# XuyangBai/PointDSC

Hardware: NVIDIA H100
Metric: correspondence-sets/sec (PointDSC.forward, N=1000, B=256) (higher is better)
Workload: dtype fp16 hi/lo split (3 products) with f32 accumulate

## Files before the change

pointdsc_b200/csrc/nsm.cu:

```cuda
#include <cuda_fp16.h>

#include "common.cuh"
#include "kernels.h"
#include "sets.cuh"
#include "warp_select.cuh"

namespace pdsc {

__global__ void gather_rows_kernel(const float* __restrict__ normed, const int32_t* __restrict__ seeds,
                                   float* __restrict__ out, const SetDesc* __restrict__ sets) {
  const int b = blockIdx.y, s = blockIdx.x, lane = threadIdx.x;
  const SetDesc d = sets[b];
  if (s >= d.S) return;
  int idx = seeds[(size_t)d.seed0 + s];
  idx = min(max(idx, 0), d.N - 1);
  const float4 v = *reinterpret_cast<const float4*>(normed + ((size_t)d.row0 + idx) * kC + lane * 4);
  *reinterpret_cast<float4*>(out + ((size_t)d.seed0 + s) * kC + lane * 4) = v;
}
void launch_gather_rows(const float* normed, const int32_t* seeds, float* out, int B, int N, int S, cudaStream_t st,
                        const SetDesc* sets) {
  if (S <= 0) return;
  gather_rows_kernel<<<dim3(S, B), 32, 0, st>>>(normed, seeds, out, sets);
}


__global__ void __launch_bounds__(256) knn_select_kernel(const float* __restrict__ dist, int32_t* __restrict__ knn_idx,
                                                         const SetDesc* __restrict__ sets, int nsets, int rows, int warps_per_cta,
                                                         int NPmax, int Pmax) {
  extern __shared__ __align__(16) unsigned char knn_smem[];
  const int lane = threadIdx.x & 31, warp = threadIdx.x >> 5;
  const int row = blockIdx.x * warps_per_cta + warp;
  if (row >= rows) return;
  const SetDesc sd = sets[find_set(nsets, row, [&](int b) { return sets[b].seed0; })];
  const int s = row - sd.seed0, N = sd.N, k = sd.k;
  int P = 2;
  while (P < k + 1) P <<= 1;
  const float* d = dist + sd.dist0 + (size_t)s * N;
  int32_t* out = knn_idx + sd.knn0 + (size_t)s * k;
  const int NP = (N + 31) & ~31;
  const size_t per_warp = (size_t)NPmax * 4 + 1024 + (size_t)Pmax * 8;
  unsigned char* base = knn_smem + (size_t)warp * per_warp;
  unsigned long long* sel = reinterpret_cast<unsigned long long*>(base);
  uint32_t* hist = reinterpret_cast<uint32_t*>(base + (size_t)Pmax * 8);
  uint32_t* keys = hist + 256;
  if ((N & 3) == 0 && (reinterpret_cast<uintptr_t>(d) & 15) == 0) {
    const uint32_t kbase = (uint32_t)__cvta_generic_to_shared(keys);
    for (int j4 = lane; j4 < (N >> 2); j4 += 32)
      asm volatile("cp.async.cg.shared.global [%0], [%1], 16;" ::"r"(kbase + (uint32_t)j4 * 16u), "l"(d + 4 * j4) : "memory");
    asm volatile("cp.async.wait_all;" ::: "memory");
  } else {
    for (int j0 = lane; j0 < N; j0 += 256) {
      float t[8];
#pragma unroll
      for (int q = 0; q < 8; ++q) t[q] = (j0 + 32 * q < N) ? d[j0 + 32 * q] : 0.f;
#pragma unroll
      for (int q = 0; q < 8; ++q)
        if (j0 + 32 * q < N) keys[j0 + 32 * q] = __float_as_uint(t[q]);
    }
  }
  __syncwarp();
  for (int j = lane; j < NP; j += 32) keys[j] = j < N ? dist_key32(__uint_as_float(keys[j])) : 0xFFFFFFFFu;
  __syncwarp();
  warp_select_sorted(keys, hist, sel, N, NP, k + 1, P, lane);
  for (int r = 1 + lane; r <= k; r += 32) {
    const unsigned long long v = sel[r];
    out[r - 1] = (v == ~0ull || (uint32_t)(v >> 32) == 0xFFFFFFFFu) ? 0 : (int32_t)(v & 0xFFFFFFFFull);
  }
}

void launch_knn_select(const float* dist, int32_t* knn_idx, int B, int N, int S, int k, cudaStream_t st,
                       const SetDesc* sets, int total_seeds) {
  if (S <= 0) return;
  const int rows = total_seeds;
  int P = 2;
  while (P < k + 1) P <<= 1;
  const int NP = (N + 31) & ~31;
  const size_t per_warp = (size_t)NP * 4 + 1024 + (size_t)P * 8;
  int warps = (int)((200 * 1024) / per_warp);
  warps = warps > 8 ? 8 : (warps < 1 ? 1 : warps);
  const int smem = (int)(per_warp * warps);
  ensure_dynamic_smem(reinterpret_cast<const void*>(knn_select_kernel), smem);
  knn_select_kernel<<<(rows + warps - 1) / warps, warps * 32, smem, st>>>(dist, knn_idx, sets, B, rows, warps, NP, P);
}

__device__ __forceinline__ void cp_async_16(uint32_t dst_smem, const void* src) {
  asm volatile("cp.async.cg.shared.global [%0], [%1], 16;" ::"r"(dst_smem), "l"(src) : "memory");
}
__device__ __forceinline__ void cp_async_wait_all() { asm volatile("cp.async.wait_all;" ::: "memory"); }

template <int WPS>
__device__ __forceinline__ void seed_group_sync() {
  if (WPS == 1) __syncwarp();
  else __syncthreads();
}

template <int WPS, int RI, int CW>
__device__ __forceinline__ uint32_t power_iteration_regs(const float* M, int ms, int k, float* v, float* red, float* it_out,
                                                         int iters, int tg) {
  constexpr int RG = 8 * WPS;
  const int lane = tg & 31, warp = tg >> 5;
  const int rg = tg >> 2, cq = tg & 3;
  const int CQ = (k + 3) >> 2;
  const int c_lo = cq * CQ, c_hi = min(k, c_lo + CQ);
  float m[RI][CW], vq[CW], vrow[RI];
#pragma unroll
  for (int i = 0; i < RI; ++i) {
    const int row = rg + RG * i;
#pragma unroll
    for (int c = 0; c < CW; ++c) m[i][c] = (row < k && c_lo + c < c_hi) ? M[row * ms + c_lo + c] : 0.f;
    vrow[i] = 1.0f;
  }
#pragma unroll
  for (int c = 0; c < CW; ++c) vq[c] = (c_lo + c < c_hi) ? 1.0f : 0.f;
  uint32_t mask = 0u;
  for (int t = 0; t < iters; ++t) {
    float u[RI], ss = 0.f;
#pragma unroll
    for (int i = 0; i < RI; ++i) {
      float p = 0.f;
#pragma unroll
      for (int c = 0; c < CW; ++c) p = fmaf(m[i][c], vq[c], p);
      p += __shfl_xor_sync(0xffffffffu, p, 1);
      p += __shfl_xor_sync(0xffffffffu, p, 2);
      u[i] = p;
      ss += (rg + RG * i < k) ? p * p : 0.f;
    }
    ss += __shfl_xor_sync(0xffffffffu, ss, 4);
    ss += __shfl_xor_sync(0xffffffffu, ss, 8);
    ss += __shfl_xor_sync(0xffffffffu, ss, 16);
    if (WPS > 1) {
      if (lane == 0) red[warp] = ss;
      __syncthreads();
      ss = ((red[0] + red[1]) + red[2]) + red[3];
    }
    const float nrm = sqrtf(ss) + 1e-6f;
    bool ok = true;
#pragma unroll
    for (int i = 0; i < RI; ++i) {
      const int row = rg + RG * i;
      const float vn = u[i] / nrm;
      ok = ok && (row >= k || fabsf(vn - vrow[i]) <= 1e-8f + 1e-5f * fabsf(vrow[i]));
      vrow[i] = vn;
      if (row < k && cq == 0) {
        v[row] = vn;
        it_out[(size_t)t * k + row] = vn;
      }
    }
    bool all_ok = __all_sync(0xffffffffu, ok);
    if (WPS > 1) {
      if (lane == 0) red[4 + warp] = all_ok ? 1.f : 0.f;
      __syncthreads();
      all_ok = (red[4] + red[5] + red[6] + red[7]) == 4.f;
    } else {
      __syncwarp();
    }
    if (all_ok) mask |= (1u << t);
#pragma unroll
    for (int c = 0; c < CW; ++c) vq[c] = (c_lo + c < c_hi) ? v[c_lo + c] : 0.f;
    if (WPS == 1) __syncwarp();
  }
  return mask;
}

template <int WPS>
__global__ void __launch_bounds__(WPS == 1 ? 256 : 128) nsm_power_kernel(
    const float* __restrict__ normed, const float* __restrict__ src, const float* __restrict__ tgt,
    const int32_t* __restrict__ knn_idx, float* __restrict__ iterates, uint32_t* __restrict__ conv_mask,
    float* __restrict__ compat_out, const SetDesc* sets, int k_lo, int k_hi, int iters, float sigma2, float sigmad2,
    int mask_stride, int groups_per_cta, int per_group_floats) {
  const float rc_sigma2 = 1.0f / sigma2, rc_sigmad2 = 1.0f / sigmad2;
  extern __shared__ __align__(16) float sm[];
  constexpr int TS = 32 * WPS;
  const int lane = threadIdx.x & 31, warp = threadIdx.x >> 5;
  const int group = (WPS == 1) ? warp : 0;
  const int tg = (WPS == 1) ? lane : (int)threadIdx.x;
  const int b = blockIdx.y;
  const SetDesc d = sets[b];
  const int N = d.N, S = d.S, k = d.k;
  if (k < k_lo || k > k_hi) return;
  const int s = blockIdx.x * groups_per_cta + group;
  if (s >= S) return;
  const int ms = k | 1;
  const int kp = (k + 3) & ~3;
  float* F = sm + (size_t)group * per_group_floats;
  float* M = F + (size_t)kp * 32;
  float* pa = M + (size_t)k * ms;
  float* pb = pa + k * 3;
  float* v = pb + k * 3;
  int* idx = reinterpret_cast<int*>(v + k);
  float* red = reinterpret_cast<float*>(idx + k);
  const size_t nb0 = (size_t)d.knn0 + (size_t)s * k;

  for (int a = tg; a < k; a += TS) {
    int j = knn_idx[nb0 + a];
    j = min(max(j, 0), N - 1);
    idx[a] = j;
    const float* ps = src + ((size_t)d.row0 + j) * 3;
    const float* pt = tgt + ((size_t)d.row0 + j) * 3;
    pa[a * 3 + 0] = ps[0]; pa[a * 3 + 1] = ps[1]; pa[a * 3 + 2] = ps[2];
    pb[a * 3 + 0] = pt[0]; pb[a * 3 + 1] = pt[1]; pb[a * 3 + 2] = pt[2];
    v[a] = 1.0f;
    M[a * ms + a] = 0.0f;
  }
  seed_group_sync<WPS>();

  const int nb = kp >> 2;
  const int nblk = nb * (nb + 1) / 2;
  constexpr int kMaxRounds = 2;
  const uint32_t f_base = (uint32_t)__cvta_generic_to_shared(F);
  for (int r0 = 0; r0 * TS < nblk; r0 += kMaxRounds) {
    int bA[kMaxRounds], bB[kMaxRounds];
    float acc[kMaxRounds][4][4];
#pragma unroll
    for (int r = 0; r < kMaxRounds; ++r) {
      const int t = tg + TS * (r0 + r);
      int A = 0, rem = t < nblk ? t : 0;
      while (rem >= nb - A) { rem -= nb - A; ++A; }
      bA[r] = A; bB[r] = A + rem;
#pragma unroll
      for (int i = 0; i < 4; ++i)
#pragma unroll
        for (int j = 0; j < 4; ++j) acc[r][i][j] = 0.f;
    }
#pragma unroll 1
    for (int quarter = 0; quarter < 4; ++quarter) {
      const int q = tg & 7;
      for (int a = tg >> 3; a < kp; a += TS / 8) {
        const uint32_t dst = f_base + (uint32_t)((a * 32 + ((q ^ ((a >> 2) & 7)) << 2)) * 4);
        if (a < k) cp_async_16(dst, normed + ((size_t)d.row0 + idx[a]) * kC + quarter * 32 + q * 4);
        else *reinterpret_cast<float4*>(F + a * 32 + ((q ^ ((a >> 2) & 7)) << 2)) = make_float4(0.f, 0.f, 0.f, 0.f);
      }
      cp_async_wait_all();
      seed_group_sync<WPS>();
#pragma unroll
      for (int r = 0; r < kMaxRounds; ++r) {
        if (tg + TS * (r0 + r) < nblk) {
          const float* xa = F + (size_t)(4 * bA[r]) * 32;
          const float* yb = F + (size_t)(4 * bB[r]) * 32;
          const int sx = bA[r] & 7, sy = bB[r] & 7;
#pragma unroll 2
          for (int cc = 0; cc < 8; ++cc) {
            float4 x[4], y[4];
#pragma unroll
            for (int i = 0; i < 4; ++i) {
              x[i] = *reinterpret_cast<const float4*>(xa + i * 32 + ((cc ^ sx) << 2));
              y[i] = *reinterpret_cast<const float4*>(yb + i * 32 + ((cc ^ sy) << 2));
            }
#pragma unroll
            for (int i = 0; i < 4; ++i)
#pragma unroll
              for (int j = 0; j < 4; ++j) {
                acc[r][i][j] = fmaf(x[i].x, y[j].x, acc[r][i][j]);
                acc[r][i][j] = fmaf(x[i].y, y[j].y, acc[r][i][j]);
                acc[r][i][j] = fmaf(x[i].z, y[j].z, acc[r][i][j]);
                acc[r][i][j] = fmaf(x[i].w, y[j].w, acc[r][i][j]);
              }
          }
        }
      }
      seed_group_sync<WPS>();
    }
#pragma unroll
    for (int r = 0; r < kMaxRounds; ++r) {
      if (tg + TS * (r0 + r) < nblk) {
#pragma unroll
        for (int i = 0; i < 4; ++i)
#pragma unroll
          for (int j = 0; j < 4; ++j) {
            const int a = 4 * bA[r] + i, c = 4 * bB[r] + j;
            if (a < c && c < k) {
              const float fm = fmaxf(__fsub_rn(1.0f, div_by_const(__fsub_rn(1.0f, acc[r][i][j]), sigma2, rc_sigma2)), 0.0f);
              const float la = length3_pow(pa[a * 3] - pa[c * 3], pa[a * 3 + 1] - pa[c * 3 + 1], pa[a * 3 + 2] - pa[c * 3 + 2]);
              const float lb = length3_pow(pb[a * 3] - pb[c * 3], pb[a * 3 + 1] - pb[c * 3 + 1], pb[a * 3 + 2] - pb[c * 3 + 2]);
              const float val = __fmul_rn(fm, consistency_rc(__fsub_rn(la, lb), sigmad2, rc_sigmad2));
              M[a * ms + c] = val;
              M[c * ms + a] = val;
            }
          }
      }
    }
  }
  seed_group_sync<WPS>();
  const size_t nb1 = (size_t)sets[b].knn0 + (size_t)(s * k);
  if (compat_out) {
    float* dst = compat_out + nb1 * k;
    for (int t = tg; t < k * k; t += TS) dst[t] = M[(t / k) * ms + (t % k)];
  }

  uint32_t mask = 0u;
  float* it_out = iterates + nb1 * iters;
  if constexpr (WPS == 1) {
    mask = power_iteration_regs<1, 5, 10>(M, ms, k, v, red, it_out, iters, tg);
  } else {
    constexpr int RG = 32, RI = kMaxK / RG;
    const int rg = tg >> 2, cq = tg & 3;
    const int CQ = (k + 3) >> 2;
    const int c_lo = cq * CQ, c_hi = min(k, c_lo + CQ);
    float vrow[RI];
#pragma unroll
    for (int i = 0; i < RI; ++i) vrow[i] = 1.0f;
    for (int t = 0; t < iters; ++t) {
      float u[RI], ss = 0.f;
#pragma unroll
      for (int i = 0; i < RI; ++i) {
        const int row = rg + RG * i;
        float p = 0.f;
        if (row < k) {
          const float* mr = M + (size_t)row * ms;
          for (int c = c_lo; c < c_hi; ++c) p = fmaf(mr[c], v[c], p);
        }
        p += __shfl_xor_sync(0xffffffffu, p, 1);
        p += __shfl_xor_sync(0xffffffffu, p, 2);
        u[i] = p;
        ss += (row < k) ? p * p : 0.f;
      }
      ss += __shfl_xor_sync(0xffffffffu, ss, 4);
      ss += __shfl_xor_sync(0xffffffffu, ss, 8);
      ss += __shfl_xor_sync(0xffffffffu, ss, 16);
      if (lane == 0) red[warp] = ss;
      __syncthreads();
      ss = ((red[0] + red[1]) + red[2]) + red[3];
      const float nrm = sqrtf(ss) + 1e-6f;
      bool ok = true;
      __syncthreads();
#pragma unroll
      for (int i = 0; i < RI; ++i) {
        const int row = rg + RG * i;
        const float vn = u[i] / nrm;
        ok = ok && (row >= k || fabsf(vn - vrow[i]) <= 1e-8f + 1e-5f * fabsf(vrow[i]));
        vrow[i] = vn;
        if (row < k && cq == 0) {
          v[row] = vn;
          it_out[(size_t)t * k + row] = vn;
        }
      }
      bool all_ok = __all_sync(0xffffffffu, ok);
      if (lane == 0) red[4 + warp] = all_ok ? 1.f : 0.f;
      __syncthreads();
      all_ok = (red[4] + red[5] + red[6] + red[7]) == 4.f;
      if (all_ok) mask |= (1u << t);
    }
  }
  if (tg == 0) atomicAnd(conv_mask + (size_t)b * mask_stride, mask);
}

__device__ __forceinline__ void mma_f16_16816(float (&d)[4], uint32_t a0, uint32_t a1, uint32_t a2, uint32_t a3, uint32_t b0,
                                              uint32_t b1) {
  asm volatile("mma.sync.aligned.m16n8k16.row.col.f32.f16.f16.f32 {%0, %1, %2, %3}, {%4, %5, %6, %7}, {%8, %9}, {%0, %1, %2, %3};"
               : "+f"(d[0]), "+f"(d[1]), "+f"(d[2]), "+f"(d[3])
               : "r"(a0), "r"(a1), "r"(a2), "r"(a3), "r"(b0), "r"(b1));
}
__device__ __forceinline__ void split_f16_pair(float a, float b, uint32_t& hi, uint32_t& lo) {
  const __half2 h = __floats2half2_rn(a, b);
  const float2 f = __half22float2(h);
  const __half2 l = __floats2half2_rn(a - f.x, b - f.y);
  hi = *reinterpret_cast<const uint32_t*>(&h);
  lo = *reinterpret_cast<const uint32_t*>(&l);
}

template <int ROWS>
__device__ __forceinline__ void stage_neighbours(const int32_t* __restrict__ knn_idx, const float* __restrict__ src,
                                                 const float* __restrict__ tgt, const SetDesc& d, size_t nb0, int ms, float* P,
                                                 float* v, int* idx, float* M, int tid, int nthreads) {
  for (int a = tid; a < ROWS; a += nthreads) {
    int j = -1;
    float sx = 0.f, sy = 0.f, sz = 0.f, tx = 0.f, ty = 0.f, tz = 0.f;
    if (a < d.k) {
      j = knn_idx[nb0 + a];
      j = min(max(j, 0), d.N - 1);
      const float* ps = src + ((size_t)d.row0 + j) * 3;
      const float* pt = tgt + ((size_t)d.row0 + j) * 3;
      sx = ps[0]; sy = ps[1]; sz = ps[2];
      tx = pt[0]; ty = pt[1]; tz = pt[2];
      M[a * ms + a] = 0.0f;
    }
    idx[a] = j;
    P[a] = sx; P[ROWS + a] = sy; P[2 * ROWS + a] = sz;
    P[3 * ROWS + a] = tx; P[4 * ROWS + a] = ty; P[5 * ROWS + a] = tz;
    v[a] = 1.0f;
  }
// ... 289 lines not shown
```

pointdsc_b200/csrc/warp_select.cuh:

```cuda
#pragma once
#include <stdint.h>

#include "common.cuh"

namespace pdsc {

__device__ __forceinline__ uint32_t dist_key32(float d) {
  uint32_t u = __float_as_uint(d);
  if (d != d) return 0xFFFFFFFFu;
  if ((u & 0x7FFFFFFFu) == 0u) u = 0u;
  return u ^ ((u & 0x80000000u) ? 0xFFFFFFFFu : 0x80000000u);
}

__device__ __forceinline__ void warp_select_sorted(uint32_t* keys, uint32_t* hist, unsigned long long* sel, int N, int NP, int want,
                                                   int P, int lane) {
  uint32_t kmin = 0xFFFFFFFFu, kmax = 0u;
  for (int j = lane; j < N; j += 32) {
    const uint32_t key = keys[j];
    kmin = min(kmin, key); kmax = max(kmax, key);
  }
  kmin = __reduce_min_sync(0xffffffffu, kmin);
  kmax = __reduce_max_sync(0xffffffffu, kmax);
  const uint32_t lt_mask = (1u << lane) - 1u;
  uint32_t prefix = 0u, T;
  int need = want;
  if (kmin == kmax) {
    T = kmin;
  } else {
    int hi_bit = 31 - __clz(kmin ^ kmax);
    prefix = (hi_bit == 31) ? 0u : (kmin >> (hi_bit + 1)) << (hi_bit + 1);
#pragma unroll 1
    while (hi_bit >= 0) {
      const int width = hi_bit + 1 < 8 ? hi_bit + 1 : 8;
      const int shift = hi_bit + 1 - width;
      const uint32_t dmask = (1u << width) - 1u;
#pragma unroll
      for (int q = 0; q < 8; ++q) hist[lane * 8 + q] = 0u;
      __syncwarp();
      for (int j = lane; j < NP; j += 32) {
        const uint32_t v = keys[j];
        const bool in = (hi_bit == 31) || ((v >> (hi_bit + 1)) == (prefix >> (hi_bit + 1)));
        if (in && j < N) atomicAdd(&hist[(v >> shift) & dmask], 1u);
      }
      __syncwarp();
      uint32_t c[8], lane_sum = 0u;
#pragma unroll
      for (int q = 0; q < 8; ++q) { c[q] = hist[lane * 8 + q]; lane_sum += c[q]; }
      uint32_t incl = lane_sum;
#pragma unroll
      for (int o = 1; o < 32; o <<= 1) {
        const uint32_t t = __shfl_up_sync(0xffffffffu, incl, o);
        if (lane >= o) incl += t;
      }
      const uint32_t excl = incl - lane_sum;
      const bool mine = excl < (uint32_t)need && (uint32_t)need <= incl;
      uint32_t digit = 0u, rem = 0u;
      if (mine) {
        uint32_t cum = excl;
#pragma unroll
        for (int q = 0; q < 8; ++q) {
          if (cum < (uint32_t)need && (uint32_t)need <= cum + c[q]) { digit = (uint32_t)(lane * 8 + q); rem = (uint32_t)need - cum; }
          cum += c[q];
        }
      }
      const int srcl = __ffs(__ballot_sync(0xffffffffu, mine)) - 1;
      digit = __shfl_sync(0xffffffffu, digit, srcl);
      need = (int)__shfl_sync(0xffffffffu, rem, srcl);
      prefix |= digit << shift;
      hi_bit = shift - 1;
      __syncwarp();
    }
    T = prefix;
  }
  int out = 0, eq_seen = 0;
  for (int j0 = 0; j0 < NP; j0 += 32) {
    const uint32_t v = keys[j0 + lane];
    const bool eq = v == T && (j0 + lane < N);
    const uint32_t beq = __ballot_sync(0xffffffffu, eq);
    const bool take = (j0 + lane < N) && ((v < T) || (eq && eq_seen + __popc(beq & lt_mask) < need));
    const uint32_t bt = __ballot_sync(0xffffffffu, take);
    if (take) sel[out + __popc(bt & lt_mask)] = ((unsigned long long)v << 32) | (unsigned)(j0 + lane);
    out += __popc(bt);
    eq_seen += __popc(beq);
  }
  for (int i = out + lane; i < P; i += 32) sel[i] = ~0ull;
  __syncwarp();
  for (int kk = 2; kk <= P; kk <<= 1) {
    for (int jj = kk >> 1; jj > 0; jj >>= 1) {
      for (int t = lane; t < (P >> 1); t += 32) {
        const int i = ((t & ~(jj - 1)) << 1) | (t & (jj - 1));
        const int ixj = i | jj;
        const unsigned long long a = sel[i], c2 = sel[ixj];
        const bool asc = (i & kk) == 0;
        if ((a > c2) == asc) { sel[i] = c2; sel[ixj] = a; }
      }
      __syncwarp();
    }
  }
}

}
```

pointdsc_b200/csrc/select_refine.cu:

```cuda
#include <cmath>

#include "common.cuh"
#include "kernels.h"
#include "sets.cuh"
#include "svd3.cuh"
#include "weighted_kabsch.cuh"

namespace pdsc {

__device__ __forceinline__ float residual(const float* T, float x, float y, float z, float tx, float ty, float tz) {
  const float px = fmaf(T[0], x, fmaf(T[1], y, T[2] * z)) + T[3];
  const float py = fmaf(T[4], x, fmaf(T[5], y, T[6] * z)) + T[7];
  const float pz = fmaf(T[8], x, fmaf(T[9], y, T[10] * z)) + T[11];
  const float dx = px - tx, dy = py - ty, dz = pz - tz;
  return sqrtf(dx * dx + dy * dy + dz * dz);
}

constexpr int kHypChunk = 1024;
__global__ void __launch_bounds__(256) seed_hypotheses_kernel(
    const float* __restrict__ src, const float* __restrict__ tgt, const int32_t* __restrict__ knn_idx,
    const float* __restrict__ iterates, const uint32_t* __restrict__ conv_mask, const float* __restrict__ seed_trans_in,
    float* __restrict__ seed_trans, int32_t* __restrict__ inlier_counts, unsigned long long* __restrict__ best_key,
    float* __restrict__ eig_out, int32_t* __restrict__ power_iters, const SetDesc* __restrict__ sets, int iters, float d2_lim,
    int mask_stride) {
  __shared__ __align__(8) float pts_s[6][kHypChunk];
  const int b = blockIdx.y;
  const SetDesc d = sets[b];
  const int N = d.N, S = d.S, k = d.k;
  if ((int)blockIdx.x * 8 >= S) return;
  const int lane = threadIdx.x & 31, warp = threadIdx.x >> 5;
  const int s_raw = blockIdx.x * 8 + warp;
  const bool active = s_raw < S;
  const int s = active ? s_raw : S - 1;
  const size_t row = (size_t)d.seed0 + s;
  const size_t nb0 = (size_t)d.knn0 + (size_t)s * k;
  const float* ps = src + (size_t)d.row0 * 3;
  const float* pt = tgt + (size_t)d.row0 * 3;

  const uint32_t m = conv_mask[(size_t)b * mask_stride] & ((iters >= 32) ? 0xFFFFFFFFu : ((1u << iters) - 1u));
  const int t_exit = m ? (__ffs(m) - 1) : (iters - 1);
  if (active && s == 0 && lane == 0 && power_iters) power_iters[b] = t_exit + 1;

  float T[12];
  if (seed_trans_in) {
#pragma unroll
    for (int i = 0; i < 12; ++i) T[i] = seed_trans_in[row * 16 + i];
  } else {
    constexpr int kPer = kMaxK / 32;
    float w[kPer], ax[kPer], ay[kPer], az[kPer], bx[kPer], by[kPer], bz[kPer];
    float wsum = 0.f;
#pragma unroll
    for (int q = 0; q < kPer; ++q) {
      const int a = lane + q * 32;
      w[q] = 0.f; ax[q] = ay[q] = az[q] = bx[q] = by[q] = bz[q] = 0.f;
      if (a < k) {
        float e = iterates[nb0 * iters + (size_t)t_exit * k + a];
        if (eig_out && active) eig_out[nb0 + a] = e;
        w[q] = e;
        int j = knn_idx[nb0 + a];
        j = min(max(j, 0), N - 1);
        ax[q] = ps[(size_t)j * 3]; ay[q] = ps[(size_t)j * 3 + 1]; az[q] = ps[(size_t)j * 3 + 2];
        bx[q] = pt[(size_t)j * 3]; by[q] = pt[(size_t)j * 3 + 1]; bz[q] = pt[(size_t)j * 3 + 2];
      }
      wsum += w[q];
    }
    wsum = warp_sum(wsum);
    const float wden = wsum + 1e-6f;
    float sw = 0.f, sax = 0.f, say = 0.f, saz = 0.f, sbx = 0.f, sby = 0.f, sbz = 0.f;
#pragma unroll
    for (int q = 0; q < kPer; ++q) {
      w[q] = w[q] / wden;
      if (w[q] < 0.f) w[q] = 0.f;
      sw += w[q];
      sax = fmaf(w[q], ax[q], sax); say = fmaf(w[q], ay[q], say); saz = fmaf(w[q], az[q], saz);
      sbx = fmaf(w[q], bx[q], sbx); sby = fmaf(w[q], by[q], sby); sbz = fmaf(w[q], bz[q], sbz);
    }
    sw = warp_sum(sw);
    sax = warp_sum(sax); say = warp_sum(say); saz = warp_sum(saz);
    sbx = warp_sum(sbx); sby = warp_sum(sby); sbz = warp_sum(sbz);
    const float den = sw + 1e-6f;
    const float cax = sax / den, cay = say / den, caz = saz / den;
    const float cbx = sbx / den, cby = sby / den, cbz = sbz / den;
    float H[9];
#pragma unroll
    for (int i = 0; i < 9; ++i) H[i] = 0.f;
#pragma unroll
    for (int q = 0; q < kPer; ++q) {
      const float mx = ax[q] - cax, my = ay[q] - cay, mz = az[q] - caz;
      const float nx = (bx[q] - cbx) * w[q], ny = (by[q] - cby) * w[q], nz = (bz[q] - cbz) * w[q];
      H[0] = fmaf(mx, nx, H[0]); H[1] = fmaf(mx, ny, H[1]); H[2] = fmaf(mx, nz, H[2]);
      H[3] = fmaf(my, nx, H[3]); H[4] = fmaf(my, ny, H[4]); H[5] = fmaf(my, nz, H[5]);
      H[6] = fmaf(mz, nx, H[6]); H[7] = fmaf(mz, ny, H[7]); H[8] = fmaf(mz, nz, H[8]);
    }
#pragma unroll
    for (int i = 0; i < 9; ++i) H[i] = warp_sum(H[i]);
    float R[9];
    kabsch_rotation(H, R);
    T[0] = R[0]; T[1] = R[1]; T[2] = R[2];  T[3] = cbx - (R[0] * cax + R[1] * cay + R[2] * caz);
    T[4] = R[3]; T[5] = R[4]; T[6] = R[5];  T[7] = cby - (R[3] * cax + R[4] * cay + R[5] * caz);
    T[8] = R[6]; T[9] = R[7]; T[10] = R[8]; T[11] = cbz - (R[6] * cax + R[7] * cay + R[8] * caz);
  }
  if (lane < 16 && active) {
    float val = (lane == 15) ? 1.0f : 0.0f;
#pragma unroll
    for (int i = 0; i < 12; ++i)
      if (lane == i) val = T[i];
    seed_trans[row * 16 + lane] = val;
  }

  int cnt = 0;
  for (int j0 = 0; j0 < N; j0 += kHypChunk) {
    __syncthreads();
    for (int f = threadIdx.x; f < 3 * kHypChunk; f += 256) {
      const int j = f / 3, c = f - 3 * j;
      const bool have = j0 + j < N;
      pts_s[c][j] = have ? ps[(size_t)(j0 + j) * 3 + c] : 0.f;
      pts_s[3 + c][j] = have ? pt[(size_t)(j0 + j) * 3 + c] : INFINITY;
    }
    __syncthreads();
    const int lim = min(kHypChunk, (N - j0 + 1) & ~1);
    for (int j = 2 * lane; j < lim; j += 64) {
      const float2 x = *reinterpret_cast<const float2*>(&pts_s[0][j]), y = *reinterpret_cast<const float2*>(&pts_s[1][j]),
                   z = *reinterpret_cast<const float2*>(&pts_s[2][j]);
      const float2 tx = *reinterpret_cast<const float2*>(&pts_s[3][j]), ty = *reinterpret_cast<const float2*>(&pts_s[4][j]),
                   tz = *reinterpret_cast<const float2*>(&pts_s[5][j]);
      float2 px = make_float2(__fmul_rn(T[2], z.x), __fmul_rn(T[2], z.y));
      float2 py = make_float2(__fmul_rn(T[6], z.x), __fmul_rn(T[6], z.y));
      float2 pz = make_float2(__fmul_rn(T[10], z.x), __fmul_rn(T[10], z.y));
      ffma2(px.x, px.y, T[1], y.x, y.y); ffma2(px.x, px.y, T[0], x.x, x.y);
      ffma2(py.x, py.y, T[5], y.x, y.y); ffma2(py.x, py.y, T[4], x.x, x.y);
      ffma2(pz.x, pz.y, T[9], y.x, y.y); ffma2(pz.x, pz.y, T[8], x.x, x.y);
      const float2 dx = make_float2(__fsub_rn(__fadd_rn(px.x, T[3]), tx.x), __fsub_rn(__fadd_rn(px.y, T[3]), tx.y));
      const float2 dy = make_float2(__fsub_rn(__fadd_rn(py.x, T[7]), ty.x), __fsub_rn(__fadd_rn(py.y, T[7]), ty.y));
      const float2 dz = make_float2(__fsub_rn(__fadd_rn(pz.x, T[11]), tz.x), __fsub_rn(__fadd_rn(pz.y, T[11]), tz.y));
      const float2 d2 = ffma2_pair(dz, dz, ffma2_pair(dy, dy, fmul2(dx, dx)));
      cnt += (d2.x < d2_lim ? 1 : 0) + (d2.y < d2_lim ? 1 : 0);
    }
  }
  if (!active) return;
  cnt = warp_sum(cnt);
  if (lane == 0) {
    if (inlier_counts) inlier_counts[row] = cnt;
    atomicMax(best_key + b, ((unsigned long long)(unsigned)cnt << 32) | (unsigned)(0xFFFFFFFFu - (unsigned)s));
  }
}

void launch_seed_hypotheses(const float* src, const float* tgt, const int32_t* knn_idx, const float* iterates,
                            const uint32_t* conv_mask, const float* seed_trans_in, float* seed_trans,
                            int32_t* inlier_counts, unsigned long long* best_key, float* eig_out, int32_t* power_iters,
                            int B, int N, int S, int k, int iters, float inlier_threshold, int mask_stride,
                            cudaStream_t st, const SetDesc* sets) {
  if (S <= 0) return;
  float d2_lim = inlier_threshold * inlier_threshold;
  while (std::sqrt(d2_lim) >= inlier_threshold && d2_lim > 0.f) d2_lim = std::nextafter(d2_lim, 0.0f);
  while (std::sqrt(d2_lim) < inlier_threshold) d2_lim = std::nextafter(d2_lim, INFINITY);
  seed_hypotheses_kernel<<<dim3((S + 7) / 8, B), 256, 0, st>>>(src, tgt, knn_idx, iterates, conv_mask, seed_trans_in,
                                                              seed_trans, inlier_counts, best_key, eig_out, power_iters, sets,
                                                              iters, d2_lim, mask_stride);
}

__global__ void __launch_bounds__(kRefThreads) select_refine_kernel(
    const float* __restrict__ src, const float* __restrict__ tgt, const float* __restrict__ seed_trans,
    const unsigned long long* __restrict__ best_key, float* __restrict__ final_trans, float* __restrict__ final_labels,
    float* __restrict__ init_trans_out, int32_t* __restrict__ best_out, int32_t* __restrict__ refine_solves, const SetDesc* __restrict__ sets,
    float thr, float rthr, int max_refine) {
  __shared__ float T[12];
  __shared__ double red[(kRefThreads / 32) * 10];
  __shared__ double tot[10];
  const int b = blockIdx.x, tid = threadIdx.x;
  const SetDesc d = sets[b];
  const int N = d.N, S = d.S;
  const float* ps = src + (size_t)d.row0 * 3;
  const float* pt = tgt + (size_t)d.row0 * 3;

  int best = 0;
  if (S > 0) {
    best = (int)(0xFFFFFFFFu - (unsigned)(best_key[b] & 0xFFFFFFFFull));
    best = min(max(best, 0), S - 1);
  }
  if (tid < 12) T[tid] = (S > 0) ? seed_trans[((size_t)d.seed0 + best) * 16 + tid] : ((tid % 5 == 0) ? 1.f : 0.f);
  __syncthreads();
  if (tid < 16 && init_trans_out) init_trans_out[(size_t)b * 16 + tid] = (tid < 12) ? T[tid] : (tid == 15 ? 1.f : 0.f);
  if (tid == 0 && best_out) best_out[b] = best;

  for (int j = tid; final_labels && j < N; j += kRefThreads) {
    const float r = residual(T, ps[(size_t)j * 3], ps[(size_t)j * 3 + 1], ps[(size_t)j * 3 + 2], pt[(size_t)j * 3],
                             pt[(size_t)j * 3 + 1], pt[(size_t)j * 3 + 2]);
    final_labels[(size_t)d.row0 + j] = (r < thr) ? 1.0f : 0.0f;
  }

  long long prev = 0;
  int solves = 0;
  for (int it = 0; it < max_refine; ++it) {
    auto weight = [&](int, float ax, float ay, float az, float bx, float by, float bz, float& w) {
      const float d = residual(T, ax, ay, az, bx, by, bz);
      if (!(d < rthr)) return false;
      const float q = d / rthr;
      w = 1.0f / (1.0f + q * q);
      return true;
    };
    kabsch_centroid_sums(ps, pt, N, weight, red, tot);
    const long long cnt = (long long)(tot[0] + 0.5);
    if (cnt == prev) break;
    prev = cnt;
    const float den = (float)tot[1] + 1e-6f;
    const float cax = (float)tot[2] / den, cay = (float)tot[3] / den, caz = (float)tot[4] / den;
    const float cbx = (float)tot[5] / den, cby = (float)tot[6] / den, cbz = (float)tot[7] / den;
    __syncthreads();
    kabsch_solve(ps, pt, N, weight, cax, cay, caz, cbx, cby, cbz, red, tot, T);
    ++solves;
    __syncthreads();
  }
  if (tid < 16) final_trans[(size_t)b * 16 + tid] = (tid < 12) ? T[tid] : (tid == 15 ? 1.f : 0.f);
  if (tid == 0 && refine_solves) refine_solves[b] = solves;
}

void launch_select_refine(const float* src, const float* tgt, const float* seed_trans,
                          const unsigned long long* best_key, float* final_trans, float* final_labels,
                          float* init_trans_out, int32_t* best_out, int32_t* refine_solves, int B, int N, int S,
                          float inlier_threshold, float refine_threshold, int max_refine, cudaStream_t st,
                          const SetDesc* sets) {
  select_refine_kernel<<<B, kRefThreads, 0, st>>>(src, tgt, seed_trans, best_key, final_trans, final_labels,
                                                  init_trans_out, best_out, refine_solves, sets, inlier_threshold,
                                                  refine_threshold, max_refine);
}

}
```

Before: 16800.

## Prefilter kNN candidates with per-group minima threshold before radix select

The kNN select kernel now computes per-lane-slot minima over 256 strided groups while converting distances to keys. It radix-selects the (k+1)-th smallest of those 256 minima to get an upper bound threshold, then compacts only keys at or below it into a candidate buffer and bitonic-sorts that. This replaces the multi-pass radix histogram over all N keys with one pass over 256 values plus a single compaction pass. If too many candidates pass (more than 2P), it falls back to the original full select. The candidate buffer per warp grows to 16*P bytes, which can reduce warps per CTA.

```diff
diff --git a/pointdsc_b200/csrc/nsm.cu b/pointdsc_b200/csrc/nsm.cu
--- a/pointdsc_b200/csrc/nsm.cu
+++ b/pointdsc_b200/csrc/nsm.cu
@@ -23,6 +23,9 @@
   gather_rows_kernel<<<dim3(S, B), 32, 0, st>>>(normed, seeds, out, sets);
 }
 
+
+constexpr int kKnnGroups = 256;
+__host__ __device__ constexpr size_t knn_cand_bytes(int P) { return (size_t)P * 16 > 1024 ? (size_t)P * 16 : 1024; }
 
 __global__ void __launch_bounds__(256) knn_select_kernel(const float* __restrict__ dist, int32_t* __restrict__ knn_idx,
                                                          const SetDesc* __restrict__ sets, int nsets, int rows, int warps_per_cta,
@@ -38,10 +41,12 @@
   const float* d = dist + sd.dist0 + (size_t)s * N;
   int32_t* out = knn_idx + sd.knn0 + (size_t)s * k;
   const int NP = (N + 31) & ~31;
-  const size_t per_warp = (size_t)NPmax * 4 + 1024 + (size_t)Pmax * 8;
+  const size_t cand_bytes = knn_cand_bytes(Pmax);
+  const size_t per_warp = (size_t)NPmax * 4 + 1024 + cand_bytes;
   unsigned char* base = knn_smem + (size_t)warp * per_warp;
   unsigned long long* sel = reinterpret_cast<unsigned long long*>(base);
-  uint32_t* hist = reinterpret_cast<uint32_t*>(base + (size_t)Pmax * 8);
+  uint32_t* gmins = reinterpret_cast<uint32_t*>(base);
+  uint32_t* hist = reinterpret_cast<uint32_t*>(base + cand_bytes);
   uint32_t* keys = hist + 256;
   if ((N & 3) == 0 && (reinterpret_cast<uintptr_t>(d) & 15) == 0) {
     const uint32_t kbase = (uint32_t)__cvta_generic_to_shared(keys);
@@ -59,9 +64,47 @@
     }
   }
   __syncwarp();
-  for (int j = lane; j < NP; j += 32) keys[j] = j < N ? dist_key32(__uint_as_float(keys[j])) : 0xFFFFFFFFu;
+  uint32_t gmin[kKnnGroups / 32];
+#pragma unroll
+  for (int q = 0; q < kKnnGroups / 32; ++q) gmin[q] = 0xFFFFFFFFu;
+  for (int j0 = 0; j0 < NP; j0 += kKnnGroups) {
+#pragma unroll
+    for (int q = 0; q < kKnnGroups / 32; ++q) {
+      const int j = j0 + 32 * q + lane;
+      if (j < NP) {
+        const uint32_t key = j < N ? dist_key32(__uint_as_float(keys[j])) : 0xFFFFFFFFu;
+        keys[j] = key;
+        gmin[q] = min(gmin[q], key);
+      }
+    }
+  }
+#pragma unroll
+  for (int q = 0; q < kKnnGroups / 32; ++q) gmins[32 * q + lane] = gmin[q];
   __syncwarp();
-  warp_select_sorted(keys, hist, sel, N, NP, k + 1, P, lane);
+  int need;
+  const uint32_t T1 = warp_radix_kth(gmins, hist, kKnnGroups, kKnnGroups, k + 1, lane, need);
+  __syncwarp();
+  const uint32_t lt_mask = (1u << lane) - 1u;
+  const int cap = 2 * P;
+  int C = 0;
+  for (int j0 = 0; j0 < NP; j0 += 32) {
+    const uint32_t v = keys[j0 + lane];
+    const bool take = (j0 + lane < N) && v <= T1;
+    const uint32_t bt = __ballot_sync(0xffffffffu, take);
+    const int at = C + __popc(bt & lt_mask);
+    if (take && at < cap) sel[at] = ((unsigned long long)v << 32) | (unsigned)(j0 + lane);
+    C += __popc(bt);
+  }
+  if (C <= cap) {
+    int P2 = P;
+    while (P2 < C) P2 <<= 1;
+    for (int i = C + lane; i < P2; i += 32) sel[i] = ~0ull;
+    __syncwarp();
+    warp_bitonic_sort(sel, P2, lane);
+  } else {
+    __syncwarp();
+    warp_select_sorted(keys, hist, sel, N, NP, k + 1, P, lane);
+  }
   for (int r = 1 + lane; r <= k; r += 32) {
     const unsigned long long v = sel[r];
     out[r - 1] = (v == ~0ull || (uint32_t)(v >> 32) == 0xFFFFFFFFu) ? 0 : (int32_t)(v & 0xFFFFFFFFull);
@@ -75,7 +118,7 @@
   int P = 2;
   while (P < k + 1) P <<= 1;
   const int NP = (N + 31) & ~31;
-  const size_t per_warp = (size_t)NP * 4 + 1024 + (size_t)P * 8;
+  const size_t per_warp = (size_t)NP * 4 + 1024 + knn_cand_bytes(P);
   int warps = (int)((200 * 1024) / per_warp);
   warps = warps > 8 ? 8 : (warps < 1 ? 1 : warps);
   const int smem = (int)(per_warp * warps);
diff --git a/pointdsc_b200/csrc/warp_select.cuh b/pointdsc_b200/csrc/warp_select.cuh
--- a/pointdsc_b200/csrc/warp_select.cuh
+++ b/pointdsc_b200/csrc/warp_select.cuh
@@ -12,8 +12,8 @@
   return u ^ ((u & 0x80000000u) ? 0xFFFFFFFFu : 0x80000000u);
 }
 
-__device__ __forceinline__ void warp_select_sorted(uint32_t* keys, uint32_t* hist, unsigned long long* sel, int N, int NP, int want,
-                                                   int P, int lane) {
+__device__ __forceinline__ uint32_t warp_radix_kth(const uint32_t* keys, uint32_t* hist, int N, int NP, int want, int lane,
+                                                   int& need_out) {
   uint32_t kmin = 0xFFFFFFFFu, kmax = 0u;
   for (int j = lane; j < N; j += 32) {
     const uint32_t key = keys[j];
@@ -21,7 +21,6 @@
   }
   kmin = __reduce_min_sync(0xffffffffu, kmin);
   kmax = __reduce_max_sync(0xffffffffu, kmax);
-  const uint32_t lt_mask = (1u << lane) - 1u;
   uint32_t prefix = 0u, T;
   int need = want;
   if (kmin == kmax) {
@@ -72,19 +71,11 @@
     }
     T = prefix;
   }
-  int out = 0, eq_seen = 0;
-  for (int j0 = 0; j0 < NP; j0 += 32) {
-    const uint32_t v = keys[j0 + lane];
-    const bool eq = v == T && (j0 + lane < N);
-    const uint32_t beq = __ballot_sync(0xffffffffu, eq);
-    const bool take = (j0 + lane < N) && ((v < T) || (eq && eq_seen + __popc(beq & lt_mask) < need));
-    const uint32_t bt = __ballot_sync(0xffffffffu, take);
-    if (take) sel[out + __popc(bt & lt_mask)] = ((unsigned long long)v << 32) | (unsigned)(j0 + lane);
-    out += __popc(bt);
-    eq_seen += __popc(beq);
-  }
-  for (int i = out + lane; i < P; i += 32) sel[i] = ~0ull;
-  __syncwarp();
+  need_out = need;
+  return T;
+}
+
+__device__ __forceinline__ void warp_bitonic_sort(unsigned long long* sel, int P, int lane) {
   for (int kk = 2; kk <= P; kk <<= 1) {
     for (int jj = kk >> 1; jj > 0; jj >>= 1) {
       for (int t = lane; t < (P >> 1); t += 32) {
@@ -99,4 +90,25 @@
   }
 }
 
+__device__ __forceinline__ void warp_select_sorted(uint32_t* keys, uint32_t* hist, unsigned long long* sel, int N, int NP, int want,
+                                                   int P, int lane) {
+  const uint32_t lt_mask = (1u << lane) - 1u;
+  int need;
+  const uint32_t T = warp_radix_kth(keys, hist, N, NP, want, lane, need);
+  int out = 0, eq_seen = 0;
+  for (int j0 = 0; j0 < NP; j0 += 32) {
+    const uint32_t v = keys[j0 + lane];
+    const bool eq = v == T && (j0 + lane < N);
+    const uint32_t beq = __ballot_sync(0xffffffffu, eq);
+    const bool take = (j0 + lane < N) && ((v < T) || (eq && eq_seen + __popc(beq & lt_mask) < need));
+    const uint32_t bt = __ballot_sync(0xffffffffu, take);
+    if (take) sel[out + __popc(bt & lt_mask)] = ((unsigned long long)v << 32) | (unsigned)(j0 + lane);
+    out += __popc(bt);
+    eq_seen += __popc(beq);
+  }
+  for (int i = out + lane; i < P; i += 32) sel[i] = ~0ull;
+  __syncwarp();
+  warp_bitonic_sort(sel, P, lane);
 }
+
+}
```

Result: no change. 16810 (median of 6 runs) (+0.1%).

## Process 32 seeds per block, reuse staged points, and batch Kabsch SVDs per lane

Applied to the files above, without the earlier changes.

Each block now handles up to 32 seeds instead of 8, so every staged point chunk in shared memory serves four seeds per warp and global reloads drop. The per-seed weighted covariance is still reduced one warp per seed, but the 3x3 Kabsch SVDs run one seed per lane in warp 0, which removes the redundant warp-wide SVD. The first chunk load is issued before the covariance work, and launch bounds now request 4 blocks per SM. In exchange there are fewer blocks, and the serial SVD in one warp can stall the whole block.

```diff
diff --git a/pointdsc_b200/csrc/select_refine.cu b/pointdsc_b200/csrc/select_refine.cu
--- a/pointdsc_b200/csrc/select_refine.cu
+++ b/pointdsc_b200/csrc/select_refine.cu
@@ -17,131 +17,177 @@
 }
 
 constexpr int kHypChunk = 1024;
-__global__ void __launch_bounds__(256) seed_hypotheses_kernel(
+constexpr int kHypSeeds = 32;
+__global__ void __launch_bounds__(256, 4) seed_hypotheses_kernel(
     const float* __restrict__ src, const float* __restrict__ tgt, const int32_t* __restrict__ knn_idx,
     const float* __restrict__ iterates, const uint32_t* __restrict__ conv_mask, const float* __restrict__ seed_trans_in,
     float* __restrict__ seed_trans, int32_t* __restrict__ inlier_counts, unsigned long long* __restrict__ best_key,
     float* __restrict__ eig_out, int32_t* __restrict__ power_iters, const SetDesc* __restrict__ sets, int iters, float d2_lim,
     int mask_stride) {
   __shared__ __align__(8) float pts_s[6][kHypChunk];
+  __shared__ float hc_s[15][kHypSeeds];
+  __shared__ float T_s[kHypSeeds][13];
   const int b = blockIdx.y;
   const SetDesc d = sets[b];
   const int N = d.N, S = d.S, k = d.k;
-  if ((int)blockIdx.x * 8 >= S) return;
+  if (S <= 0) return;
+  const int runs = (S + kHypSeeds - 1) / kHypSeeds;
+  const int per = (S + runs - 1) / runs;
+  const int s0 = (int)blockIdx.x * per;
+  if (s0 >= S) return;
+  const int ns = min(per, S - s0);
   const int lane = threadIdx.x & 31, warp = threadIdx.x >> 5;
-  const int s_raw = blockIdx.x * 8 + warp;
-  const bool active = s_raw < S;
-  const int s = active ? s_raw : S - 1;
-  const size_t row = (size_t)d.seed0 + s;
-  const size_t nb0 = (size_t)d.knn0 + (size_t)s * k;
   const float* ps = src + (size_t)d.row0 * 3;
   const float* pt = tgt + (size_t)d.row0 * 3;
 
   const uint32_t m = conv_mask[(size_t)b * mask_stride] & ((iters >= 32) ? 0xFFFFFFFFu : ((1u << iters) - 1u));
   const int t_exit = m ? (__ffs(m) - 1) : (iters - 1);
-  if (active && s == 0 && lane == 0 && power_iters) power_iters[b] = t_exit + 1;
-
-  float T[12];
-  if (seed_trans_in) {
-#pragma unroll
-    for (int i = 0; i < 12; ++i) T[i] = seed_trans_in[row * 16 + i];
-  } else {
-    constexpr int kPer = kMaxK / 32;
-    float w[kPer], ax[kPer], ay[kPer], az[kPer], bx[kPer], by[kPer], bz[kPer];
-    float wsum = 0.f;
-#pragma unroll
-    for (int q = 0; q < kPer; ++q) {
-      const int a = lane + q * 32;
-      w[q] = 0.f; ax[q] = ay[q] = az[q] = bx[q] = by[q] = bz[q] = 0.f;
-      if (a < k) {
-        float e = iterates[nb0 * iters + (size_t)t_exit * k + a];
-        if (eig_out && active) eig_out[nb0 + a] = e;
-        w[q] = e;
-        int j = knn_idx[nb0 + a];
-        j = min(max(j, 0), N - 1);
-        ax[q] = ps[(size_t)j * 3]; ay[q] = ps[(size_t)j * 3 + 1]; az[q] = ps[(size_t)j * 3 + 2];
-        bx[q] = pt[(size_t)j * 3]; by[q] = pt[(size_t)j * 3 + 1]; bz[q] = pt[(size_t)j * 3 + 2];
-      }
-      wsum += w[q];
-    }
-    wsum = warp_sum(wsum);
-    const float wden = wsum + 1e-6f;
-    float sw = 0.f, sax = 0.f, say = 0.f, saz = 0.f, sbx = 0.f, sby = 0.f, sbz = 0.f;
-#pragma unroll
-    for (int q = 0; q < kPer; ++q) {
-      w[q] = w[q] / wden;
-      if (w[q] < 0.f) w[q] = 0.f;
-      sw += w[q];
-      sax = fmaf(w[q], ax[q], sax); say = fmaf(w[q], ay[q], say); saz = fmaf(w[q], az[q], saz);
-      sbx = fmaf(w[q], bx[q], sbx); sby = fmaf(w[q], by[q], sby); sbz = fmaf(w[q], bz[q], sbz);
-    }
-    sw = warp_sum(sw);
-    sax = warp_sum(sax); say = warp_sum(say); saz = warp_sum(saz);
-    sbx = warp_sum(sbx); sby = warp_sum(sby); sbz = warp_sum(sbz);
-    const float den = sw + 1e-6f;
-    const float cax = sax / den, cay = say / den, caz = saz / den;
-    const float cbx = sbx / den, cby = sby / den, cbz = sbz / den;
-    float H[9];
-#pragma unroll
-    for (int i = 0; i < 9; ++i) H[i] = 0.f;
-#pragma unroll
-    for (int q = 0; q < kPer; ++q) {
-      const float mx = ax[q] - cax, my = ay[q] - cay, mz = az[q] - caz;
-      const float nx = (bx[q] - cbx) * w[q], ny = (by[q] - cby) * w[q], nz = (bz[q] - cbz) * w[q];
-      H[0] = fmaf(mx, nx, H[0]); H[1] = fmaf(mx, ny, H[1]); H[2] = fmaf(mx, nz, H[2]);
-      H[3] = fmaf(my, nx, H[3]); H[4] = fmaf(my, ny, H[4]); H[5] = fmaf(my, nz, H[5]);
-      H[6] = fmaf(mz, nx, H[6]); H[7] = fmaf(mz, ny, H[7]); H[8] = fmaf(mz, nz, H[8]);
-    }
-#pragma unroll
-    for (int i = 0; i < 9; ++i) H[i] = warp_sum(H[i]);
-    float R[9];
-    kabsch_rotation(H, R);
-    T[0] = R[0]; T[1] = R[1]; T[2] = R[2];  T[3] = cbx - (R[0] * cax + R[1] * cay + R[2] * caz);
-    T[4] = R[3]; T[5] = R[4]; T[6] = R[5];  T[7] = cby - (R[3] * cax + R[4] * cay + R[5] * caz);
-    T[8] = R[6]; T[9] = R[7]; T[10] = R[8]; T[11] = cbz - (R[6] * cax + R[7] * cay + R[8] * caz);
-  }
-  if (lane < 16 && active) {
-    float val = (lane == 15) ? 1.0f : 0.0f;
-#pragma unroll
-    for (int i = 0; i < 12; ++i)
-      if (lane == i) val = T[i];
-    seed_trans[row * 16 + lane] = val;
-  }
-
-  int cnt = 0;
-  for (int j0 = 0; j0 < N; j0 += kHypChunk) {
-    __syncthreads();
+  if (blockIdx.x == 0 && threadIdx.x == 0 && power_iters) power_iters[b] = t_exit + 1;
+
+  auto stage = [&](int j0) {
     for (int f = threadIdx.x; f < 3 * kHypChunk; f += 256) {
       const int j = f / 3, c = f - 3 * j;
       const bool have = j0 + j < N;
       pts_s[c][j] = have ? ps[(size_t)(j0 + j) * 3 + c] : 0.f;
       pts_s[3 + c][j] = have ? pt[(size_t)(j0 + j) * 3 + c] : INFINITY;
     }
-    __syncthreads();
+  };
+  stage(0);
+
+  if (!seed_trans_in) {
+    for (int i = warp; i < ns; i += 8) {
+      const int s = s0 + i;
+      const size_t nb0 = (size_t)d.knn0 + (size_t)s * k;
+      constexpr int kPer = kMaxK / 32;
+      float w[kPer], ax[kPer], ay[kPer], az[kPer], bx[kPer], by[kPer], bz[kPer];
+      float wsum = 0.f;
+#pragma unroll
+      for (int q = 0; q < kPer; ++q) {
+        const int a = lane + q * 32;
+        w[q] = 0.f; ax[q] = ay[q] = az[q] = bx[q] = by[q] = bz[q] = 0.f;
+        if (a < k) {
+          float e = iterates[nb0 * iters + (size_t)t_exit * k + a];
+          if (eig_out) eig_out[nb0 + a] = e;
+          w[q] = e;
+          int j = knn_idx[nb0 + a];
+          j = min(max(j, 0), N - 1);
+          ax[q] = ps[(size_t)j * 3]; ay[q] = ps[(size_t)j * 3 + 1]; az[q] = ps[(size_t)j * 3 + 2];
+          bx[q] = pt[(size_t)j * 3]; by[q] = pt[(size_t)j * 3 + 1]; bz[q] = pt[(size_t)j * 3 + 2];
+        }
+        wsum += w[q];
+      }
+      wsum = warp_sum(wsum);
+      const float wden = wsum + 1e-6f;
+      float sw = 0.f, sax = 0.f, say = 0.f, saz = 0.f, sbx = 0.f, sby = 0.f, sbz = 0.f;
+#pragma unroll
+      for (int q = 0; q < kPer; ++q) {
+        w[q] = w[q] / wden;
+        if (w[q] < 0.f) w[q] = 0.f;
+        sw += w[q];
+        sax = fmaf(w[q], ax[q], sax); say = fmaf(w[q], ay[q], say); saz = fmaf(w[q], az[q], saz);
+        sbx = fmaf(w[q], bx[q], sbx); sby = fmaf(w[q], by[q], sby); sbz = fmaf(w[q], bz[q], sbz);
+      }
+      sw = warp_sum(sw);
+      sax = warp_sum(sax); say = warp_sum(say); saz = warp_sum(saz);
+      sbx = warp_sum(sbx); sby = warp_sum(sby); sbz = warp_sum(sbz);
+      const float den = sw + 1e-6f;
+      const float cax = sax / den, cay = say / den, caz = saz / den;
+      const float cbx = sbx / den, cby = sby / den, cbz = sbz / den;
+      float H[9];
+#pragma unroll
+      for (int c = 0; c < 9; ++c) H[c] = 0.f;
+#pragma unroll
+      for (int q = 0; q < kPer; ++q) {
+        const float mx = ax[q] - cax, my = ay[q] - cay, mz = az[q] - caz;
+        const float nx = (bx[q] - cbx) * w[q], ny = (by[q] - cby) * w[q], nz = (bz[q] - cbz) * w[q];
+        H[0] = fmaf(mx, nx, H[0]); H[1] = fmaf(mx, ny, H[1]); H[2] = fmaf(mx, nz, H[2]);
+        H[3] = fmaf(my, nx, H[3]); H[4] = fmaf(my, ny, H[4]); H[5] = fmaf(my, nz, H[5]);
+        H[6] = fmaf(mz, nx, H[6]); H[7] = fmaf(mz, ny, H[7]); H[8] = fmaf(mz, nz, H[8]);
+      }
+#pragma unroll
+      for (int c = 0; c < 9; ++c) H[c] = warp_sum(H[c]);
+      if (lane == 0) {
+#pragma unroll
+        for (int c = 0; c < 9; ++c) hc_s[c][i] = H[c];
+        hc_s[9][i] = cax; hc_s[10][i] = cay; hc_s[11][i] = caz;
+        hc_s[12][i] = cbx; hc_s[13][i] = cby; hc_s[14][i] = cbz;
+      }
+    }
+  }
+  __syncthreads();
+  if (warp == 0 && lane < ns) {
+    const size_t row = (size_t)d.seed0 + s0 + lane;
+    float T[12];
+    if (seed_trans_in) {
+#pragma unroll
+      for (int c = 0; c < 12; ++c) T[c] = seed_trans_in[row * 16 + c];
+    } else {
+      float H[9], R[9];
+#pragma unroll
+      for (int c = 0; c < 9; ++c) H[c] = hc_s[c][lane];
+      const float cax = hc_s[9][lane], cay = hc_s[10][lane], caz = hc_s[11][lane];
+      const float cbx = hc_s[12][lane], cby = hc_s[13][lane], cbz = hc_s[14][lane];
+      kabsch_rotation(H, R);
+      T[0] = R[0]; T[1] = R[1]; T[2] = R[2];  T[3] = cbx - (R[0] * cax + R[1] * cay + R[2] * caz);
+      T[4] = R[3]; T[5] = R[4]; T[6] = R[5];  T[7] = cby - (R[3] * cax + R[4] * cay + R[5] * caz);
+      T[8] = R[6]; T[9] = R[7]; T[10] = R[8]; T[11] = cbz - (R[6] * cax + R[7] * cay + R[8] * caz);
+    }
+#pragma unroll
+    for (int c = 0; c < 12; ++c) T_s[lane][c] = T[c];
+  }
+  __syncthreads();
+  for (int e = threadIdx.x; e < ns * 16; e += 256) {
+    const int i = e >> 4, c = e & 15;
+    seed_trans[((size_t)d.seed0 + s0 + i) * 16 + c] = (c < 12) ? T_s[i][c] : ((c == 15) ? 1.0f : 0.0f);
+  }
+
+  constexpr int kSeedsPerWarp = kHypSeeds / 8;
+  int cnt[kSeedsPerWarp];
+#pragma unroll
+  for (int q = 0; q < kSeedsPerWarp; ++q) cnt[q] = 0;
+  for (int j0 = 0;;) {
     const int lim = min(kHypChunk, (N - j0 + 1) & ~1);
-    for (int j = 2 * lane; j < lim; j += 64) {
-      const float2 x = *reinterpret_cast<const float2*>(&pts_s[0][j]), y = *reinterpret_cast<const float2*>(&pts_s[1][j]),
-                   z = *reinterpret_cast<const float2*>(&pts_s[2][j]);
-      const float2 tx = *reinterpret_cast<const float2*>(&pts_s[3][j]), ty = *reinterpret_cast<const float2*>(&pts_s[4][j]),
-                   tz = *reinterpret_cast<const float2*>(&pts_s[5][j]);
-      float2 px = make_float2(__fmul_rn(T[2], z.x), __fmul_rn(T[2], z.y));
-      float2 py = make_float2(__fmul_rn(T[6], z.x), __fmul_rn(T[6], z.y));
-      float2 pz = make_float2(__fmul_rn(T[10], z.x), __fmul_rn(T[10], z.y));
-      ffma2(px.x, px.y, T[1], y.x, y.y); ffma2(px.x, px.y, T[0], x.x, x.y);
-      ffma2(py.x, py.y, T[5], y.x, y.y); ffma2(py.x, py.y, T[4], x.x, x.y);
-      ffma2(pz.x, pz.y, T[9], y.x, y.y); ffma2(pz.x, pz.y, T[8], x.x, x.y);
-      const float2 dx = make_float2(__fsub_rn(__fadd_rn(px.x, T[3]), tx.x), __fsub_rn(__fadd_rn(px.y, T[3]), tx.y));
-      const float2 dy = make_float2(__fsub_rn(__fadd_rn(py.x, T[7]), ty.x), __fsub_rn(__fadd_rn(py.y, T[7]), ty.y));
-      const float2 dz = make_float2(__fsub_rn(__fadd_rn(pz.x, T[11]), tz.x), __fsub_rn(__fadd_rn(pz.y, T[11]), tz.y));
-      const float2 d2 = ffma2_pair(dz, dz, ffma2_pair(dy, dy, fmul2(dx, dx)));
-      cnt += (d2.x < d2_lim ? 1 : 0) + (d2.y < d2_lim ? 1 : 0);
-    }
-  }
-  if (!active) return;
-  cnt = warp_sum(cnt);
-  if (lane == 0) {
-    if (inlier_counts) inlier_counts[row] = cnt;
-    atomicMax(best_key + b, ((unsigned long long)(unsigned)cnt << 32) | (unsigned)(0xFFFFFFFFu - (unsigned)s));
+#pragma unroll
+    for (int q = 0; q < kSeedsPerWarp; ++q) {
+      const int i = warp + 8 * q;
+      if (i >= ns) break;
+      float T[12];
+#pragma unroll
+      for (int c = 0; c < 12; ++c) T[c] = T_s[i][c];
+      for (int j = 2 * lane; j < lim; j += 64) {
+        const float2 x = *reinterpret_cast<const float2*>(&pts_s[0][j]), y = *reinterpret_cast<const float2*>(&pts_s[1][j]),
+                     z = *reinterpret_cast<const float2*>(&pts_s[2][j]);
+        const float2 tx = *reinterpret_cast<const float2*>(&pts_s[3][j]), ty = *reinterpret_cast<const float2*>(&pts_s[4][j]),
+                     tz = *reinterpret_cast<const float2*>(&pts_s[5][j]);
+        float2 px = make_float2(__fmul_rn(T[2], z.x), __fmul_rn(T[2], z.y));
+        float2 py = make_float2(__fmul_rn(T[6], z.x), __fmul_rn(T[6], z.y));
+        float2 pz = make_float2(__fmul_rn(T[10], z.x), __fmul_rn(T[10], z.y));
+        ffma2(px.x, px.y, T[1], y.x, y.y); ffma2(px.x, px.y, T[0], x.x, x.y);
+        ffma2(py.x, py.y, T[5], y.x, y.y); ffma2(py.x, py.y, T[4], x.x, x.y);
+        ffma2(pz.x, pz.y, T[9], y.x, y.y); ffma2(pz.x, pz.y, T[8], x.x, x.y);
+        const float2 dx = make_float2(__fsub_rn(__fadd_rn(px.x, T[3]), tx.x), __fsub_rn(__fadd_rn(px.y, T[3]), tx.y));
+        const float2 dy = make_float2(__fsub_rn(__fadd_rn(py.x, T[7]), ty.x), __fsub_rn(__fadd_rn(py.y, T[7]), ty.y));
+        const float2 dz = make_float2(__fsub_rn(__fadd_rn(pz.x, T[11]), tz.x), __fsub_rn(__fadd_rn(pz.y, T[11]), tz.y));
+        const float2 d2 = ffma2_pair(dz, dz, ffma2_pair(dy, dy, fmul2(dx, dx)));
+        cnt[q] += (d2.x < d2_lim ? 1 : 0) + (d2.y < d2_lim ? 1 : 0);
+      }
+    }
+    j0 += kHypChunk;
+    if (j0 >= N) break;
+    __syncthreads();
+    stage(j0);
+    __syncthreads();
+  }
+#pragma unroll
+  for (int q = 0; q < kSeedsPerWarp; ++q) {
+    const int i = warp + 8 * q;
+    if (i >= ns) break;
+    const int c = warp_sum(cnt[q]);
+    if (lane == 0) {
+      const int s = s0 + i;
+      if (inlier_counts) inlier_counts[(size_t)d.seed0 + s] = c;
+      atomicMax(best_key + b, ((unsigned long long)(unsigned)c << 32) | (unsigned)(0xFFFFFFFFu - (unsigned)s));
+    }
   }
 }
 
@@ -154,9 +200,9 @@
   float d2_lim = inlier_threshold * inlier_threshold;
   while (std::sqrt(d2_lim) >= inlier_threshold && d2_lim > 0.f) d2_lim = std::nextafter(d2_lim, 0.0f);
   while (std::sqrt(d2_lim) < inlier_threshold) d2_lim = std::nextafter(d2_lim, INFINITY);
-  seed_hypotheses_kernel<<<dim3((S + 7) / 8, B), 256, 0, st>>>(src, tgt, knn_idx, iterates, conv_mask, seed_trans_in,
-                                                              seed_trans, inlier_counts, best_key, eig_out, power_iters, sets,
-                                                              iters, d2_lim, mask_stride);
+  seed_hypotheses_kernel<<<dim3((S + kHypSeeds - 1) / kHypSeeds, B), 256, 0, st>>>(
+      src, tgt, knn_idx, iterates, conv_mask, seed_trans_in, seed_trans, inlier_counts, best_key, eig_out, power_iters, sets,
+      iters, d2_lim, mask_stride);
 }
 
 __global__ void __launch_bounds__(kRefThreads) select_refine_kernel(
```

Measured after the change: 16500 before, 16610 after (median of 6 runs). About the same (+0.7%).
